# hiroharu-kato/neural_renderer

Measured on AMD Instinct MI355X. Metric: rasterize fwd+bwd Mpixels/sec @256x256 batch=64, higher is better.
Workload: dtype f32

## Files before the change

neural_renderer_amd/csrc/nr_forward.hip:

```cpp
#include "nr_device.h"

using namespace nr;

namespace {

constexpr size_t SMALL_LAUNCH_FACES = (size_t)16384 * 32;
constexpr int SMALL_AREA = 256;
constexpr int WAVE_AREA = 4096;
constexpr unsigned long long ZEMPTY = ~0ull;
constexpr int QSHARDS = 16;
constexpr int QSTRIDE = 32;

__device__ __forceinline__ unsigned depth_key(float zp)
{
    const unsigned u = __float_as_uint(zp + 0.0f);
    return (u & 0x80000000u) ? ~u : (u | 0x80000000u);
}

__device__ __forceinline__ unsigned long long zword(float zp, unsigned fn, int epoch)
{
    const unsigned long long k = depth_key(zp);
    return epoch < 0 ? (k << 32) | fn : ((unsigned long long)(unsigned)epoch << 56) | (k << 24) | fn;
}

// ... 350 lines not shown
            const int b = i / F;
            raster_candidates(
                g, (unsigned)(i - b * F), cd.n, (int)(threadIdx.x >> 6) * 64, 256,
                [&](int k, int &x, int &y) { return cand_pixel(cd, k, S, x, y); }, queue, S, near_d, far_d,
                zbuf + (size_t)b * S * S, epoch, touched, (size_t)b * S * S);
        }
    }
    wave_raster(faces, zbuf, wave_list, cnt, qcap, nshards, F, S, near_d, far_d, queue, epoch, touched);
}

enum ShadeMode { SHADE_CUBE = 0, SHADE_UV = 1, SHADE_CORNER = 2, SHADE_UV_SMOOTH = 3 };
__device__ __forceinline__ void load_background(const float *__restrict__ background, int bg_per_batch, int b, float (&bg)[3])
{
    const float *p = background + (bg_per_batch ? 3 * b : 0);
    bg[0] = p[0];
    bg[1] = p[1];
    bg[2] = p[2];
}

template <bool TS2>
struct CubeFace {
    float fz[3], lc[3];
    const float *texture;
    bool flip;
    float4 cube[TS2 ? 6 : 1];
};

template <bool TS2, bool SHARED = false>
__device__ __forceinline__ void load_cube_face(CubeFace<TS2> &c, int b, int fi, const float *__restrict__ faces,
                                               const float *__restrict__ zbase, const float *__restrict__ textures, int F,
                                               int ts, int fix_batch_z, const FaceLight &lit)
{
    const float *face = (fix_batch_z ? faces + (size_t)b * F * 9 : zbase) + (size_t)fi * 9;
    c.fz[0] = face[2]; c.fz[1] = face[5]; c.fz[2] = face[8];
    if constexpr (TS2) {
        c.flip = false;
        c.texture = textures + ((size_t)(SHARED ? 0 : b) * F + fi) * 24;
    } else {
        c.flip = lit.light && fi >= lit.tex_faces;
        c.texture = textures + ((size_t)(SHARED ? 0 : b) * (lit.light ? lit.tex_faces : F) + (c.flip ? fi - lit.tex_faces : fi)) * ts * ts * ts * 3;
        const float *lc = lit.light ? lit.light + ((size_t)b * F + fi) * 3 : face;
        c.lc[0] = lc[0]; c.lc[1] = lc[1]; c.lc[2] = lc[2];
    }
}

__device__ __forceinline__ void load_cube(CubeFace<true> &c)
{
#pragma unroll
    for (int k = 0; k < 6; k++) c.cube[k] = reinterpret_cast<const float4 *>(c.texture)[k];
}
__device__ __forceinline__ void load_cube(CubeFace<false> &) {}

__device__ __forceinline__ float quad_elem(const float4 &q, int k) { return k == 0 ? q.x : (k == 1 ? q.y : (k == 2 ? q.z : q.w)); }

__device__ __forceinline__ void store_taps(const Taps &t, int32_t *__restrict__ sampling_index_map,
                                           float *__restrict__ sampling_weight_map, size_t i)
{
    if (sampling_index_map) {
        int4 *p = reinterpret_cast<int4 *>(sampling_index_map + 8 * i);
        p[0] = make_int4(t.isc[0], t.isc[1], t.isc[2], t.isc[3]);
        p[1] = make_int4(t.isc[4], t.isc[5], t.isc[6], t.isc[7]);
    }
    if (sampling_weight_map) {
        float4 *p = reinterpret_cast<float4 *>(sampling_weight_map + 8 * i);
        p[0] = make_float4(t.w[0], t.w[1], t.w[2], t.w[3]);
        p[1] = make_float4(t.w[4], t.w[5], t.w[6], t.w[7]);
    }
}

template <bool TS2>
__device__ __forceinline__ void shade_cube(const CubeFace<TS2> &c, const float (&w)[3], float depth, int ts, double eps,
                                           bool lit, Taps &t, float (&rgb)[3], int32_t *__restrict__ sampling_index_map = nullptr,
                                           float *__restrict__ sampling_weight_map = nullptr, size_t i = 0)
{
    compute_taps(c.fz, w, depth, ts, eps, t, c.flip);
    store_taps(t, sampling_index_map, sampling_weight_map, i);
    if constexpr (TS2) {
        rgb[0] = rgb[1] = rgb[2] = 0.0f;
#pragma unroll
        for (int pn = 0; pn < 8; pn++) {
            const int b0 = pn & 1, b1 = (pn >> 1) & 1, b2 = pn >> 2;
            const int e = (b0 * 4 + b1 * 2 + b2) * 3;
#pragma unroll
            for (int k = 0; k < 3; k++) rgb[k] += t.w[pn] * quad_elem(c.cube[(e + k) >> 2], (e + k) & 3);
        }
    } else {
        sum_taps(c.texture, t, ts * ts * ts, rgb);
    }
    if (!TS2 && lit) {
        rgb[0] *= c.lc[0];
        rgb[1] *= c.lc[1];
        rgb[2] *= c.lc[2];
    }
}

template <int MODE>
__device__ __forceinline__ void shade_pixel(size_t i, int b, int fi, float w0, float w1, float w2, float depth,
                                            const float *__restrict__ faces, const float *__restrict__ zbase,
                                            const float *__restrict__ textures, float *__restrict__ rgb_map,
                                            int32_t *__restrict__ sampling_index_map,
                                            float *__restrict__ sampling_weight_map, const float (&bg)[3],
                                            float *__restrict__ alpha_map, int F, int ts, double eps, int fix_batch_z,
                                            const FaceLight &lit, const UVShade *uv = nullptr)
{
    if (alpha_map) alpha_map[i] = (fi >= 0) ? 1.0f : 0.0f;
    if (!rgb_map) return;
    float rgb[3];
    Taps t;
    constexpr bool UV = MODE == SHADE_UV || MODE == SHADE_UV_SMOOTH;
    if (MODE == SHADE_CORNER && fi >= 0) {
        const float *face = faces + ((size_t)b * F + fi) * 9;
        const float *cc = textures + ((size_t)b * F + fi) * 9;
        const float w[3] = {w0, w1, w2}, fz[3] = {face[2], face[5], face[8]};
        float d[3];
        corner_weights(fz, w, depth, d);
#pragma unroll
        for (int c = 0; c < 3; c++) {
            rgb[c] = (cc[c] * d[0] + cc[3 + c] * d[1]) + cc[6 + c] * d[2];
            rgb[c] = rgb[c] * 1.0f + 0.0f * bg[c];
        }
    } else if (UV && fi >= 0) {
        UVSample s;
        uv_locate(*uv, fi, lit.tex_faces, faces + ((size_t)b * F + fi) * 9, w0, w1, w2, depth, eps, s);
        uv_color(*uv, s, b, rgb);
        if (MODE == SHADE_UV_SMOOTH) {
            const float *face = faces + ((size_t)b * F + fi) * 9;
            const float w[3] = {w0, w1, w2}, fz[3] = {face[2], face[5], face[8]};
            float e[3];
            corner_weights(fz, w, depth, e);
            const float *lc = lit.light + ((size_t)b * F + fi) * 9;
#pragma unroll
            for (int c = 0; c < 3; c++) rgb[c] *= (lc[c] * e[0] + lc[3 + c] * e[1]) + lc[6 + c] * e[2];
        } else {
            const float *lc = lit.light + ((size_t)b * F + fi) * 3;
            rgb[0] *= lc[0];
            rgb[1] *= lc[1];
            rgb[2] *= lc[2];
        }
#pragma unroll
        for (int k = 0; k < 3; k++) rgb[k] = rgb[k] * 1.0f + 0.0f * bg[k];
    } else if (fi >= 0) {
        CubeFace<false> c;
        load_cube_face(c, b, fi, faces, zbase, textures, F, ts, fix_batch_z, lit);
        const float w[3] = {w0, w1, w2};
        shade_cube(c, w, depth, ts, eps, lit.light != nullptr, t, rgb, sampling_index_map, sampling_weight_map, i);
#pragma unroll
        for (int k = 0; k < 3; k++) rgb[k] = rgb[k] * 1.0f + 0.0f * bg[k];
    } else {
#pragma unroll
        for (int k = 0; k < 3; k++) rgb[k] = 0.0f * 0.0f + 1.0f * bg[k];
#pragma unroll
        for (int pn = 0; pn < 8; pn++) { t.isc[pn] = 0; t.w[pn] = 0.0f; }
    }
    float *o = rgb_map + 3 * i;
    o[0] = rgb[0];
    o[1] = rgb[1];
    o[2] = rgb[2];
    if (MODE == SHADE_CUBE && fi < 0) store_taps(t, sampling_index_map, sampling_weight_map, i);
}

__global__ __launch_bounds__(256) void k_shade(const float *__restrict__ faces, const float *__restrict__ zbase,
                                               const float *__restrict__ textures,
                                               const int32_t *__restrict__ face_index_map,
                                               const float *__restrict__ weight_map,
                                               const float *__restrict__ depth_map, float *__restrict__ rgb_map,
                                               int32_t *__restrict__ sampling_index_map,
                                               float *__restrict__ sampling_weight_map,
                                               const float *__restrict__ background, int bg_per_batch,
                                               float *__restrict__ alpha_map, int F, int S, int ts, double eps,
                                               int fix_batch_z, size_t n_pixels, FaceLight lit)
{
    const size_t i = (size_t)blockIdx.x * blockDim.x + threadIdx.x;
    if (i >= n_pixels) return;
    const int b = (int)(i / ((size_t)S * S));
    float bg[3] = {0.0f, 0.0f, 0.0f};
    if (rgb_map) load_background(background, bg_per_batch, b, bg);
    const int fi = face_index_map[i];
    float w0 = 0.0f, w1 = 0.0f, w2 = 0.0f, depth = 0.0f;
    if (rgb_map && fi >= 0) { w0 = weight_map[3 * i]; w1 = weight_map[3 * i + 1]; w2 = weight_map[3 * i + 2]; depth = depth_map[i]; }
    shade_pixel<SHADE_CUBE>(i, b, fi, w0, w1, w2, depth, faces, zbase, textures, rgb_map, sampling_index_map, sampling_weight_map,
                            bg, alpha_map, F, ts, eps, fix_batch_z, lit);
}

struct ResolveArgs {
    const float *faces;
    const unsigned long long *zbuf;
    int32_t *face_index_map;
    float *weight_map, *depth_map, *face_inv_map;
    unsigned char *visible_faces;
    int F, S;
    double near_d, far_d;
    size_t n_pixels;
    const float *zbase, *textures;
    float *rgb_map;
    const float *background;
    int bg_per_batch;
    float *alpha_map;
    int ts;
    double eps;
    int fix_batch_z, epoch;
    int *queue_counters;
    FaceLight lit;
    int sparse_weights;
    const unsigned char *touched;
};
struct ResolveArgsUV : ResolveArgs {
    UVShade uv;
};
template <int MODE> using ResolveArgsOf =
    typename std::conditional<MODE == SHADE_UV || MODE == SHADE_UV_SMOOTH, ResolveArgsUV, ResolveArgs>::type;

template <int MODE, bool TS2, bool SHARED = false>
__device__ __forceinline__ void resolve_pixel(const ResolveArgsOf<MODE> &a, size_t i, unsigned long long pk, const float (&bg)[3])
{
    constexpr bool CUBE = MODE == SHADE_CUBE;
    const float *__restrict__ faces = a.faces;
    const int S = a.S, F = a.F, epoch = a.epoch;
    int fn = -1;
    float zp = (float)a.far_d, w0 = 0.0f, w1 = 0.0f, w2 = 0.0f;
    int b = 0;
    float rgb[3];
    const bool hit = epoch < 0 ? pk != ZEMPTY : (int)(pk >> 56) == epoch;
    if (hit) {
        fn = epoch < 0 ? (int)(unsigned)(pk & 0xffffffffu) : (int)(unsigned)(pk & 0xffffffu);
        const size_t SS = (size_t)S * S;
        b = (int)(i / SS);
        const int pn = (int)(i - (size_t)b * SS);
        const int py = pn / S, px = pn - py * S;
        const float *f = faces + ((size_t)b * F + fn) * 9;
        const float fv[9] = {f[0], f[1], f[2], f[3], f[4], f[5], f[6], f[7], f[8]};
        CubeFace<TS2> c;
        if (CUBE && a.rgb_map) load_cube_face<TS2, SHARED>(c, b, fn, faces, a.zbase, a.textures, F, a.ts, a.fix_batch_z, a.lit);
        FaceGeo g;
        float inv[9];
        face_geo(fv, S, g, inv);
        if (CUBE && a.rgb_map) load_cube(c);
        eval_pixel(g, pixel_center_f(px, S), pixel_center_f(py, S), (float)px, (float)py, a.near_d, a.far_d, zp, w0, w1, w2);
        if (a.face_inv_map) {
            float *o = a.face_inv_map + 9 * i;
#pragma unroll
            for (int k = 0; k < 9; k++) o[k] = inv[k];
        }
        if (CUBE && a.rgb_map) {
            Taps t;
            const float w[3] = {w0, w1, w2};
            shade_cube(c, w, zp, a.ts, a.eps, a.lit.light != nullptr, t, rgb);
#pragma unroll
            for (int k = 0; k < 3; k++) rgb[k] = rgb[k] * 1.0f + 0.0f * bg[k];
        }
    } else {
#pragma unroll
        for (int k = 0; k < 3; k++) rgb[k] = 0.0f * 0.0f + 1.0f * bg[k];
    }
    a.face_index_map[i] = fn;
    if (a.depth_map) a.depth_map[i] = zp;
    if (a.weight_map && (hit || !a.sparse_weights)) {
        float *w = a.weight_map + 3 * i;
        w[0] = w0;
        w[1] = w1;
        w[2] = w2;
    }
    if (a.face_inv_map && !hit) {
        float *o = a.face_inv_map + 9 * i;
#pragma unroll
        for (int k = 0; k < 9; k++) o[k] = 0.0f;
    }
    if (hit && a.visible_faces) a.visible_faces[(size_t)b * F + fn] = 1;
    if constexpr (CUBE) {
        if (a.alpha_map) a.alpha_map[i] = hit ? 1.0f : 0.0f;
        if (a.rgb_map) {
            float *o = a.rgb_map + 3 * i;
            o[0] = rgb[0];
            o[1] = rgb[1];
            o[2] = rgb[2];
        }
    } else if (a.rgb_map || a.alpha_map) {
        const UVShade *uv = nullptr;
        if constexpr (MODE == SHADE_UV || MODE == SHADE_UV_SMOOTH) uv = &a.uv;
        shade_pixel<MODE>(i, b, fn, w0, w1, w2, zp, faces, a.zbase, a.textures, a.rgb_map, nullptr, nullptr, bg, a.alpha_map, F,
                          a.ts, a.eps, a.fix_batch_z, a.lit, uv);
    }
}

__device__ __forceinline__ void reset_queue_counters(const ResolveArgs &a)
{
    if (blockIdx.x == 0 && threadIdx.x < QSHARDS && a.epoch >= 0) {
        a.queue_counters[threadIdx.x * QSTRIDE] = -1;
        a.queue_counters[threadIdx.x * QSTRIDE + 1] = -1;
    }
}

template <int MODE, bool SHARED = false>
__global__ __launch_bounds__(256, 8) void k_resolve(ResolveArgsOf<MODE> a)
{
    const size_t i = (size_t)blockIdx.x * blockDim.x + threadIdx.x;
    reset_queue_counters(a);
    if (i >= a.n_pixels) return;
    float bg[3] = {0.0f, 0.0f, 0.0f};
    if (a.rgb_map) load_background(a.background, a.bg_per_batch, a.bg_per_batch ? (int)(i / ((size_t)a.S * a.S)) : 0, bg);
    const bool drawn = !a.touched || a.touched[i >> 6] == (unsigned char)a.epoch;
    resolve_pixel<MODE, false, SHARED>(a, i, drawn ? a.zbuf[i] : ZEMPTY, bg);
}

template <int MODE, bool TS2 = false, bool SHARED = false>
__global__ __launch_bounds__(256, 8) void k_resolve_quads(ResolveArgsOf<MODE> a)
{
    reset_queue_counters(a);
    const size_t i = (size_t)blockIdx.x * 256 + threadIdx.x, i0 = (size_t)blockIdx.x * 256 + 4 * threadIdx.x;
    const size_t last = a.n_pixels - 1;
    const unsigned char ep = (unsigned char)a.epoch;
    const bool filler = threadIdx.x < 64 && i0 < a.n_pixels;
    const unsigned char tq_read = a.touched[(filler ? i0 : min(i, last)) >> 6], ti_read = a.touched[min(i, last) >> 6];
    float bg[3] = {0.0f, 0.0f, 0.0f};
    if (a.rgb_map)
        load_background(a.background, a.bg_per_batch, a.bg_per_batch ? (int)(((size_t)blockIdx.x * 256) / ((size_t)a.S * a.S)) : 0, bg);
    const unsigned char tq = filler ? tq_read : ep, ti = i < a.n_pixels ? ti_read : (unsigned char)(ep + 1);
    unsigned long long pk = ZEMPTY;
    if (ti == ep) pk = a.zbuf[i];
    if (tq != ep) {
        reinterpret_cast<int4 *>(a.face_index_map)[i0 >> 2] = make_int4(-1, -1, -1, -1);
        const float zf = (float)a.far_d;
        if (a.depth_map) reinterpret_cast<float4 *>(a.depth_map)[i0 >> 2] = make_float4(zf, zf, zf, zf);
        const float4 zero = make_float4(0.0f, 0.0f, 0.0f, 0.0f);
        if (a.weight_map && !a.sparse_weights) {
            float4 *w = reinterpret_cast<float4 *>(a.weight_map + 3 * i0);
            w[0] = zero; w[1] = zero; w[2] = zero;
        }
        if (a.face_inv_map) {
            float4 *o = reinterpret_cast<float4 *>(a.face_inv_map + 9 * i0);
#pragma unroll
            for (int k = 0; k < 9; k++) o[k] = zero;
        }
        if (a.alpha_map) reinterpret_cast<float4 *>(a.alpha_map)[i0 >> 2] = zero;
        if (a.rgb_map) {
            float c[3];
#pragma unroll
            for (int k = 0; k < 3; k++) c[k] = 0.0f * 0.0f + 1.0f * bg[k];
            float4 *o = reinterpret_cast<float4 *>(a.rgb_map + 3 * i0);
            o[0] = make_float4(c[0], c[1], c[2], c[0]);
            o[1] = make_float4(c[1], c[2], c[0], c[1]);
            o[2] = make_float4(c[2], c[0], c[1], c[2]);
        }
    }
    if (ti == ep) resolve_pixel<MODE, TS2, SHARED>(a, i, pk, bg);
}

}

NR_API int nr_version(void) { return NR_VERSION; }

NR_API const char *nr_error_string(int code)
{
    switch (code) {
        case 0: return "success";
        case NR_E_NULL: return "nr: a required pointer is NULL";
        case NR_E_SIZE: return "nr: size out of range";
        case NR_E_WORKSPACE: return "nr: workspace missing or too small";
        case NR_E_MODE: return "nr: nothing to do / inconsistent optional arguments";
        case NR_E_INDEX: return "nr: a vertex index lies outside [0, num_vertices)";
        default: return code > 0 ? hipGetErrorString((hipError_t)code) : "nr: unknown error";
    }
}

namespace {
struct FwdLayout {
    size_t zbuf_off, list_off, count_off, touch_off, total;
};
size_t queue_shard_capacity(size_t n_faces, int faces_per_wave, int nshards)
{
    const size_t per_wg = (size_t)4 * faces_per_wave, n_wg = (n_faces + per_wg - 1) / per_wg;
    return (n_wg + nshards - 1) / nshards * per_wg;
}

FwdLayout fwd_layout(int B, int F, int S)
{
    FwdLayout L;
    const size_t n = (size_t)B * F, P = (size_t)B * S * S;
    L.zbuf_off = 0;
    L.count_off = L.zbuf_off + P * sizeof(unsigned long long);
    L.list_off = align_up(L.count_off + (size_t)QSHARDS * QSTRIDE * sizeof(int), 256);
    L.touch_off = align_up(L.list_off + 2 * (n + (size_t)QSHARDS * 256) * sizeof(int), 256);
    L.total = L.touch_off + (P + 63) / 64;
    return L;
}
}

NR_API size_t nr_forward_workspace_bytes(int32_t B, int32_t F, int32_t S)
{
    if (check_sizes(B, F, S)) return 0;
    return fwd_layout(B, F, S).total;
}

namespace {
int run_forward(const float *faces, int32_t *face_index_map, float *weight_map, float *depth_map, float *face_inv_map,
                unsigned char *visible_faces, int B, int F, int S, double near, double far, void *workspace,
                size_t workspace_bytes, hipStream_t st, const float *faces_z_ref, const float *textures, float *rgb_map,
                const float *background, int bg_per_batch, float *alpha_map, int ts, double eps, int fix_batch_z,
                int flags = 0, const FaceLight &lit = FaceLight(), const UVShade *uv = nullptr, bool corner = false,
                bool corner_light = false, bool shared_cubes = false)
{
    if (!faces || !face_index_map) return NR_E_NULL;
    if (int e = check_sizes(B, F, S)) return e;
    const FwdLayout L = fwd_layout(B, F, S);
    if (!workspace || workspace_bytes < L.total) return NR_E_WORKSPACE;
    const size_t n = (size_t)B * F, P = (size_t)B * S * S;
    unsigned char *ws = (unsigned char *)workspace;
    unsigned long long *zbuf = (unsigned long long *)(ws + L.zbuf_off);
    int *n_large = (int *)(ws + L.count_off);
    int *large_list = (int *)(ws + L.list_off);

    int epoch = -1;
    if ((flags & NR_FLAG_ZBUF_EPOCH) && F < (1 << 24)) {
        epoch = (flags >> 8) & 0xff;
        if (epoch > 254) return NR_E_MODE;
    } else {
        if (int he = fill_bytes(zbuf, 0xff, P * sizeof(unsigned long long) + (size_t)QSHARDS * QSTRIDE * sizeof(int), st)) return he;
    }
    const bool small_launch = n < SMALL_LAUNCH_FACES;
    const int nshards = small_launch ? 1 : QSHARDS;
    const int qcap = (int)queue_shard_capacity(n, small_launch ? 16 : 64, nshards);
    int *wave_list = large_list + (size_t)nshards * qcap;
    unsigned char *touched = epoch >= 0 ? ws + L.touch_off : nullptr;
    {
        const bool pow2 = (S & (S - 1)) == 0, small = small_launch;
#define NR_FACE_RASTER(P, FC, G)                                                                                           \
    hipLaunchKernelGGL((k_face_raster<P, FC, G>), dim3((unsigned)((n + 4 * FC - 1) / (4 * FC))), dim3(256), 0, st, faces, zbuf, \
                       large_list, wave_list, n_large, qcap, nshards, visible_faces, (int)n, F, S, near, far, epoch, touched)
        if (small) { if (pow2) NR_FACE_RASTER(true, 16, 4); else NR_FACE_RASTER(false, 16, 4); }
        else { if (pow2) NR_FACE_RASTER(true, 64, 16); else NR_FACE_RASTER(false, 64, 16); }
#undef NR_FACE_RASTER
    }
    const unsigned queue_wgs = (unsigned)(n / 256 < 256 ? 256 : (n / 256 > 2048 ? 2048 : n / 256));
    hipLaunchKernelGGL(k_large_raster, dim3(queue_wgs), dim3(256), 0, st, faces, zbuf, large_list, wave_list, n_large, qcap, nshards,
                       F, S, near, far, epoch, touched);
    ResolveArgs ra;
    ra.faces = faces; ra.zbuf = zbuf; ra.face_index_map = face_index_map; ra.weight_map = weight_map; ra.depth_map = depth_map;
    ra.face_inv_map = face_inv_map; ra.visible_faces = visible_faces; ra.F = F; ra.S = S; ra.near_d = near; ra.far_d = far;
    ra.n_pixels = P; ra.zbase = faces_z_ref ? faces_z_ref : faces; ra.textures = textures; ra.rgb_map = rgb_map;
    ra.background = background; ra.bg_per_batch = bg_per_batch; ra.alpha_map = alpha_map; ra.ts = ts; ra.eps = eps;
    ra.fix_batch_z = fix_batch_z; ra.epoch = epoch; ra.queue_counters = n_large; ra.lit = lit;
    ra.sparse_weights = (flags & NR_FLAG_SPARSE_WEIGHT_MAP) ? 1 : 0; ra.touched = touched;
    const uintptr_t align = (uintptr_t)face_index_map | (uintptr_t)weight_map | (uintptr_t)depth_map | (uintptr_t)face_inv_map |
                            (uintptr_t)rgb_map | (uintptr_t)alpha_map;
    const bool quads = touched && S % 2 == 0 && (align & 15) == 0 && (!(rgb_map && bg_per_batch) || ((size_t)S * S) % 256 == 0);
    const dim3 grid((unsigned)((P + 255) / 256));
    if (uv) {
        ResolveArgsUV rau;
        static_cast<ResolveArgs &>(rau) = ra;
        rau.uv = *uv;
        if (corner_light) {
            if (quads) hipLaunchKernelGGL(k_resolve_quads<SHADE_UV_SMOOTH>, grid, dim3(256), 0, st, rau);
            else hipLaunchKernelGGL(k_resolve<SHADE_UV_SMOOTH>, grid, dim3(256), 0, st, rau);
        } else if (quads) {
            hipLaunchKernelGGL(k_resolve_quads<SHADE_UV>, grid, dim3(256), 0, st, rau);
        } else {
            hipLaunchKernelGGL(k_resolve<SHADE_UV>, grid, dim3(256), 0, st, rau);
        }
    } else if (corner) {
        if (quads) hipLaunchKernelGGL(k_resolve_quads<SHADE_CORNER>, grid, dim3(256), 0, st, ra);
        else hipLaunchKernelGGL(k_resolve<SHADE_CORNER>, grid, dim3(256), 0, st, ra);
    } else if (shared_cubes) {
        if (quads && rgb_map && !lit.light && ts == 2 && (float)(1.0 - eps) < 1.0f && ((uintptr_t)textures & 15) == 0)
            hipLaunchKernelGGL((k_resolve_quads<SHADE_CUBE, true, true>), grid, dim3(256), 0, st, ra);
        else if (quads) hipLaunchKernelGGL((k_resolve_quads<SHADE_CUBE, false, true>), grid, dim3(256), 0, st, ra);
        else hipLaunchKernelGGL((k_resolve<SHADE_CUBE, true>), grid, dim3(256), 0, st, ra);
    } else if (quads && rgb_map && !lit.light && ts == 2 && (float)(1.0 - eps) < 1.0f && ((uintptr_t)textures & 15) == 0) {
        hipLaunchKernelGGL((k_resolve_quads<SHADE_CUBE, true>), grid, dim3(256), 0, st, ra);
    } else if (quads) {
        hipLaunchKernelGGL(k_resolve_quads<SHADE_CUBE>, grid, dim3(256), 0, st, ra);
    } else {
        hipLaunchKernelGGL(k_resolve<SHADE_CUBE>, grid, dim3(256), 0, st, ra);
    }
    return launch_status();
}
}

NR_API int nr_forward_face_index_map(const float *faces, int32_t *face_index_map, float *weight_map, float *depth_map,
                                     float *face_inv_map, uint8_t *visible_faces, int32_t B, int32_t F, int32_t S,
                                     double near, double far, void *workspace, size_t workspace_bytes, void *stream)
{
    return run_forward(faces, face_index_map, weight_map, depth_map, face_inv_map, visible_faces, B, F, S, near, far,
                       workspace, workspace_bytes, (hipStream_t)stream, nullptr, nullptr, nullptr, nullptr, 0, nullptr, 0,
                       0.0, 0);
}

NR_API int nr_forward_rasterize(const float *faces, const float *faces_z_ref, const float *textures,
                                int32_t *face_index_map, float *weight_map, float *depth_map, float *rgb_map,
                                float *alpha_map, uint8_t *visible_faces, const float *background, int32_t bg_per_batch,
                                int32_t B, int32_t F, int32_t S, int32_t ts, double near, double far, double eps,
                                int32_t flags, void *workspace, size_t workspace_bytes, void *stream)
{
    return nr_forward_rasterize_lit(nullptr, faces, faces_z_ref, textures, face_index_map, weight_map, depth_map, rgb_map,
                                    alpha_map, visible_faces, background, bg_per_batch, B, F, S, ts, near, far, eps, flags,
                                    workspace, workspace_bytes, stream);
}

int nr::face_light_args(const nr_face_light *lit, int F, bool backward, FaceLight &out)
{
    out = FaceLight();
    if (!lit) return 0;
    if (!lit->light) return NR_E_NULL;
    if (lit->texture_faces < 1 || (lit->texture_faces != F && 2 * (int64_t)lit->texture_faces != F)) return NR_E_SIZE;
    out.light = lit->light;
    out.tex_faces = lit->texture_faces;
    if (backward) {
        out.textures = lit->textures;
        out.grad_light = lit->grad_light;
        if (out.grad_light && !out.textures) return NR_E_NULL;
    }
    return 0;
}

NR_API int nr_forward_rasterize_lit(const nr_face_light *lit, const float *faces, const float *faces_z_ref,
                                    const float *textures, int32_t *face_index_map, float *weight_map, float *depth_map,
                                    float *rgb_map, float *alpha_map, uint8_t *visible_faces, const float *background,
                                    int32_t bg_per_batch, int32_t B, int32_t F, int32_t S, int32_t ts, double near,
                                    double far, double eps, int32_t flags, void *workspace, size_t workspace_bytes,
                                    void *stream)
{
    if (rgb_map) {
        if (!textures || !background) return NR_E_NULL;
        if (ts < 2 || ts > 1024) return NR_E_SIZE;
    }
    FaceLight fl;
    if (int e = face_light_args(rgb_map ? lit : nullptr, F, false, fl)) return e;
    return run_forward(faces, face_index_map, weight_map, depth_map, nullptr, visible_faces, B, F, S, near, far,
                       workspace, workspace_bytes, (hipStream_t)stream, faces_z_ref, textures, rgb_map, background,
                       bg_per_batch, alpha_map, ts, eps, (flags & NR_FLAG_FIX_TEXTURE_BATCH_Z) ? 1 : 0, flags, fl, nullptr, false,
                       false, rgb_map && (flags & NR_FLAG_SHARED_TEXTURES));
}

int nr::uv_images_args(const nr_face_light *lit, const nr_uv_images *uv, int B, int F, FaceLight &fl, UVShade &out)
{
    out = UVShade();
    if (!lit || !uv) return NR_E_NULL;
    if (int e = face_light_args(lit, F, false, fl)) return e;
    fl.grad_light = lit->grad_light;
    if (!uv->images || !uv->image_table || !uv->faces_uv || !uv->face_image || !uv->base) return NR_E_NULL;
    if (uv->texture_size < 2 || uv->texture_size > 1024 || uv->num_images < 1 || uv->num_pixels < 1 ||
        uv->num_pixels > 0x7ffffffe)
        return NR_E_SIZE;
    if (uv->image_batch != 1 && uv->image_batch != B) return NR_E_SIZE;
    out.images = uv->images;
    out.table = uv->image_table;
    out.faces_uv = uv->faces_uv;
    out.face_image = uv->face_image;
    out.base = uv->base;
    out.ts = uv->texture_size;
    out.M = uv->num_images;
    out.P = uv->num_pixels;
    out.shared = uv->image_batch == 1 ? 1 : 0;
    return 0;
}

NR_API int nr_forward_rasterize_uv(const nr_face_light *lit, const nr_uv_images *uv, const float *faces,
                                   int32_t *face_index_map, float *weight_map, float *depth_map, float *rgb_map,
                                   float *alpha_map, uint8_t *visible_faces, const float *background, int32_t bg_per_batch,
                                   int32_t B, int32_t F, int32_t S, double near, double far, double eps, int32_t flags,
                                   void *workspace, size_t workspace_bytes, void *stream)
{
    if (!rgb_map || !background) return NR_E_NULL;
    FaceLight fl;
    UVShade us;
    if (int e = uv_images_args(lit, uv, B, F, fl, us)) return e;
    return run_forward(faces, face_index_map, weight_map, depth_map, nullptr, visible_faces, B, F, S, near, far,
                       workspace, workspace_bytes, (hipStream_t)stream, nullptr, nullptr, rgb_map, background,
                       bg_per_batch, alpha_map, us.ts, eps, 1, flags, fl, &us);
}

int nr::uv_smooth_args(const nr_corner_light *lit, const nr_uv_images *uv, int B, int F, FaceLight &fl, UVShade &out)
{
    if (!lit) return NR_E_NULL;
    const nr_face_light as_face = {lit->light, lit->texture_faces, nullptr, lit->grad_light};
    return uv_images_args(&as_face, uv, B, F, fl, out);
}

NR_API int nr_forward_rasterize_uv_smooth(const nr_corner_light *lit, const nr_uv_images *uv, const float *faces,
                                          int32_t *face_index_map, float *weight_map, float *depth_map, float *rgb_map,
                                          float *alpha_map, uint8_t *visible_faces, const float *background,
                                          int32_t bg_per_batch, int32_t B, int32_t F, int32_t S, double near, double far,
                                          double eps, int32_t flags, void *workspace, size_t workspace_bytes, void *stream)
{
    if (!rgb_map || !background) return NR_E_NULL;
    FaceLight fl;
    UVShade us;
    if (int e = uv_smooth_args(lit, uv, B, F, fl, us)) return e;
    return run_forward(faces, face_index_map, weight_map, depth_map, nullptr, visible_faces, B, F, S, near, far,
                       workspace, workspace_bytes, (hipStream_t)stream, nullptr, nullptr, rgb_map, background,
                       bg_per_batch, alpha_map, us.ts, eps, 1, flags, fl, &us, false, true);
}

NR_API int nr_forward_rasterize_corner(const float *corner_colors, const float *faces, int32_t *face_index_map,
                                       float *weight_map, float *depth_map, float *rgb_map, float *alpha_map,
                                       uint8_t *visible_faces, const float *background, int32_t bg_per_batch, int32_t B,
                                       int32_t F, int32_t S, double near, double far, int32_t flags, void *workspace,
                                       size_t workspace_bytes, void *stream)
{
    if (!corner_colors || !rgb_map || !background) return NR_E_NULL;
    return run_forward(faces, face_index_map, weight_map, depth_map, nullptr, visible_faces, B, F, S, near, far,
                       workspace, workspace_bytes, (hipStream_t)stream, nullptr, corner_colors, rgb_map, background,
                       bg_per_batch, alpha_map, 2, 0.0, 1, flags, FaceLight(), nullptr, true);
}

NR_API int nr_forward_texture_sampling(const float *faces, const float *faces_z_ref, const float *textures,
                                       const int32_t *face_index_map, const float *weight_map, const float *depth_map,
                                       float *rgb_map, int32_t *sampling_index_map, float *sampling_weight_map,
                                       const float *background, int32_t bg_per_batch, float *alpha_map, int32_t B,
                                       int32_t F, int32_t S, int32_t ts, double eps, int32_t flags, void *stream)
{
    if (!face_index_map) return NR_E_NULL;
    if (!rgb_map && !alpha_map) return NR_E_MODE;
    if (flags & NR_FLAG_SHARED_TEXTURES) return NR_E_MODE;
    if (int e = check_sizes(B, F, S)) return e;
    if (rgb_map) {
        if (!faces || !textures || !weight_map || !depth_map || !background) return NR_E_NULL;
        if (ts < 2 || ts > 1024) return NR_E_SIZE;
        if ((sampling_index_map == nullptr) != (sampling_weight_map == nullptr)) return NR_E_MODE;
    }
    const size_t n = (size_t)B * S * S;
    hipLaunchKernelGGL(k_shade, dim3((unsigned)((n + 255) / 256)), dim3(256), 0, (hipStream_t)stream, faces,
                       faces_z_ref ? faces_z_ref : faces, textures, face_index_map, weight_map, depth_map, rgb_map,
                       sampling_index_map, sampling_weight_map, background, bg_per_batch, alpha_map, F, S, ts, eps,
                       (flags & NR_FLAG_FIX_TEXTURE_BATCH_Z) ? 1 : 0, n, FaceLight());
    return launch_status();
}
```

neural_renderer_amd/csrc/nr_k6_lists.h:

```cpp

__global__ __launch_bounds__(256) void k_mark_visible(const int32_t *__restrict__ fi_map,
                                                      unsigned char *__restrict__ flags, int F, int SS, size_t P)
{
    const size_t i = (size_t)blockIdx.x * blockDim.x + threadIdx.x;
    if (i >= P) return;
    const int fi = fi_map[i];
    if (fi >= 0) flags[(i / SS) * F + fi] = 1;
}

__device__ __forceinline__ void emit_visible(int b, int fn, int pos, int F, int S, const float *__restrict__ faces,
                                             int *__restrict__ vis_list, unsigned *__restrict__ rng,
                                             double *__restrict__ scratch, int *band_count, int n_bands, int W,
                                             int *line_diff = nullptr)
{
    vis_list[(size_t)b * F + pos] = fn;
    const float *f = faces + ((size_t)b * F + fn) * 9;
    const float fs = (float)S;
    float px[3], py[3];
#pragma unroll
    for (int k = 0; k < 3; k++) { px[k] = to_pixel(f[3 * k], fs); py[k] = to_pixel(f[3 * k + 1], fs); }
    unsigned *r0 = rng + (((size_t)b * 2 + 0) * F + pos) * 3, *r1 = rng + (((size_t)b * 2 + 1) * F + pos) * 3;
#pragma unroll
    for (int e = 0; e < 3; e++) {
        const unsigned ra = edge_range(px[e], px[(e + 1) % 3], S), rb = edge_range(py[e], py[(e + 1) % 3], S);
        r0[e] = ra;
        r1[e] = rb;
#pragma unroll
        for (int axis = 0; axis < 2; axis++) {
            const unsigned r = axis ? rb : ra;
            const int lo = (int)(r & 0xffffu), hi = (int)(r >> 16);
            if (line_diff) {
                if (lo <= hi) {
                    atomicAdd(line_diff + axis * (S + 1) + lo, 1);
                    atomicAdd(line_diff + axis * (S + 1) + hi + 1, -1);
                }
                continue;
            }
            for (int band = lo / W; band * W <= hi; ++band)
                atomicAdd(band_count + axis * n_bands + band, min(hi, band * W + W - 1) - max(lo, band * W) + 1);
        }
    }
    double2 *z = reinterpret_cast<double2 *>(scratch + ((size_t)b * F + pos) * 6);
    z[0] = z[1] = z[2] = make_double2(0.0, 0.0);
}

__device__ __forceinline__ void zero_face(float *__restrict__ o)
{
#pragma unroll
    for (int k = 0; k < 9; k++) o[k] = 0.0f;
}

constexpr int VIS_CHUNK = 1024;
constexpr int SMALL_CHUNKS = 16;

__device__ __forceinline__ int chunk_flags_before(const unsigned char *flags, int b, int F, int chunk)
{
    int part = 0;
    for (int c = 0, tid = threadIdx.x; c < chunk; ++c) part += __popcll(__ballot(flags[(size_t)b * F + c * VIS_CHUNK + tid] != 0));
    return part;
}
__device__ __forceinline__ unsigned long long chunk_rank(bool v, int part, int *s_part, int *s_wcnt, int &off, int &own)
{
    const int tid = threadIdx.x, lane = tid & 63, wave = tid >> 6;
    const unsigned long long m = __ballot(v);
    if (lane == 0) { s_part[wave] = part; s_wcnt[wave] = __popcll(m); }
    __syncthreads();
    off = own = 0;
    for (int w = 0; w < VIS_CHUNK / 64; ++w) {
        off += s_part[w];
        if (w < wave) off += s_wcnt[w];
        own += s_wcnt[w];
    }
    return m;
}
__device__ __forceinline__ int chunk_rank_total(int own, const int *s_part)
{
    int base = 0;
    for (int w = 0; w < VIS_CHUNK / 64; ++w) base += s_part[w];
    return base + own;
}

__global__ __launch_bounds__(VIS_CHUNK) void k_compact_par(const unsigned char *__restrict__ flags,
                                                           int *__restrict__ vis_list, int *__restrict__ vis_count,
                                                           int *__restrict__ slot_of, int F, int n_chunks,
                                                           const float *__restrict__ faces, unsigned *__restrict__ rng,
                                                           double *__restrict__ scratch, int S,
                                                           int *__restrict__ chunk_band, int n_bands, int W,
                                                           int *__restrict__ band_cursor, float *__restrict__ zero_faces,
                                                           int zero_listed, int use_diff, int *__restrict__ ticket)
{
    extern __shared__ int s_band[];
    __shared__ int s_wcnt[VIS_CHUNK / 64];
    __shared__ int s_part[VIS_CHUNK / 64];
    const int b = blockIdx.y, chunk = blockIdx.x, tid = threadIdx.x, lane = tid & 63, wave = tid >> 6;
    for (int i = tid; i < 2 * n_bands; i += VIS_CHUNK) s_band[i] = 0;
    int *s_diff = use_diff ? s_band + 2 * n_bands : nullptr;
    if (use_diff)
        for (int i = tid; i < 2 * (S + 1); i += VIS_CHUNK) s_diff[i] = 0;
    const int part = chunk_flags_before(flags, b, F, chunk), fn = chunk * VIS_CHUNK + tid;
    const bool v = fn < F && flags[(size_t)b * F + fn] != 0;
    int off, own;
    const unsigned long long m = chunk_rank(v, part, s_part, s_wcnt, off, own);
    if (fn < F) {
        const int before = off + __popcll(m & ((1ull << lane) - 1ull));
        slot_of[(size_t)b * F + fn] = v ? before : -1;
        if (v) emit_visible(b, fn, before, F, S, faces, vis_list, rng, scratch, s_band, n_bands, W, s_diff);
        if (zero_faces && (!v || zero_listed)) zero_face(zero_faces + ((size_t)b * F + fn) * 9);
    }
    __syncthreads();
    if (use_diff) {
        const int n2 = 2 * (S + 1), per = (n2 + VIS_CHUNK - 1) / VIS_CHUNK, i0 = tid * per, i1 = min(n2, i0 + per);
        int local = 0;
        for (int i = i0; i < i1; ++i) local += s_diff[i];
        const int inc = wave_incl_scan(local, lane);
        __syncthreads();
        if (lane == 63) s_wcnt[wave] = inc;
        __syncthreads();
        int run = inc - local;
        for (int w = 0; w < wave; ++w) run += s_wcnt[w];
        for (int i = i0; i < i1; ++i) {
            run += s_diff[i];
            s_diff[i] = run;
        }
        __syncthreads();
        for (int i = tid; i < 2 * n_bands; i += VIS_CHUNK) {
            const int axis = i >= n_bands, band = i - axis * n_bands;
            int c = 0;
            for (int l = band * W; l < min(S, band * W + W); ++l) c += s_diff[axis * (S + 1) + l];
            s_band[i] = c;
        }
        __syncthreads();
    }
    int *row = chunk_band + ((size_t)b * n_chunks + chunk) * 2 * n_bands;
    for (int i = tid; i < 2 * n_bands; i += VIS_CHUNK) row[i] = s_band[i];
    if (chunk == 0)
        for (int i = tid; i < 2 * n_bands; i += VIS_CHUNK) band_cursor[(size_t)b * 2 * n_bands + i] = 0;
    if (chunk == n_chunks - 1 && tid == 0) vis_count[b] = chunk_rank_total(own, s_part);
    if (chunk == 0 && b == 0 && tid == 0) *ticket = 0;
}

__global__ __launch_bounds__(VIS_CHUNK) void k_list_visible(const unsigned char *__restrict__ flags,
                                                            int *__restrict__ vis_list, int *__restrict__ vis_count, int F,
                                                            int n_chunks)
{
    __shared__ int s_wcnt[VIS_CHUNK / 64];
    __shared__ int s_part[VIS_CHUNK / 64];
    const int b = blockIdx.y, chunk = blockIdx.x, tid = threadIdx.x, lane = tid & 63;
    const int part = chunk_flags_before(flags, b, F, chunk), fn = chunk * VIS_CHUNK + tid;
    const bool v = fn < F && flags[(size_t)b * F + fn] != 0;
    int off, own;
    const unsigned long long m = chunk_rank(v, part, s_part, s_wcnt, off, own);
    if (v) vis_list[(size_t)b * F + off + __popcll(m & ((1ull << lane) - 1ull))] = fn;
    if (chunk == n_chunks - 1 && tid == 0) vis_count[b] = chunk_rank_total(own, s_part);
}

__global__ __launch_bounds__(VIS_CHUNK) void k_count_visible(const unsigned char *__restrict__ flags,
                                                             int *__restrict__ chunk_count, int F, int n_chunks,
                                                             int *__restrict__ band_lines, int n_bands)
{
    __shared__ int s_wcnt[VIS_CHUNK / 64];
    const int b = blockIdx.y, chunk = blockIdx.x, tid = threadIdx.x, lane = tid & 63, wave = tid >> 6;
    for (int i = chunk * VIS_CHUNK + tid; i < 2 * n_bands; i += n_chunks * VIS_CHUNK) band_lines[(size_t)b * 2 * n_bands + i] = 0;
    const int fn = chunk * VIS_CHUNK + tid;
    const bool v = fn < F && flags[(size_t)b * F + fn] != 0;
    const unsigned long long m = __ballot(v);
    if (lane == 0) s_wcnt[wave] = __popcll(m);
    __syncthreads();
    if (tid == 0) {
        int tot = 0;
        for (int w = 0; w < VIS_CHUNK / 64; ++w) tot += s_wcnt[w];
        chunk_count[(size_t)b * n_chunks + chunk] = tot;
    }
}

__global__ __launch_bounds__(VIS_CHUNK) void k_compact_visible(const unsigned char *__restrict__ flags,
                                                               const int *__restrict__ chunk_count,
                                                               int *__restrict__ vis_list, int *__restrict__ vis_count,
                                                               int *__restrict__ slot_of, int F, int n_chunks,
                                                               const float *__restrict__ faces,
                                                               unsigned *__restrict__ rng, double *__restrict__ scratch,
                                                               int S, int *__restrict__ band_lines, int n_bands, int W,
                                                               int lds_counters, float *__restrict__ zero_faces,
                                                               int zero_listed)
{
    extern __shared__ int s_band[];
    __shared__ int s_wcnt[VIS_CHUNK / 64];
    __shared__ int s_part[VIS_CHUNK / 64];
    const int b = blockIdx.y, chunk = blockIdx.x, tid = threadIdx.x;
    if (lds_counters)
        for (int i = tid; i < 2 * n_bands; i += VIS_CHUNK) s_band[i] = 0;
    int part = 0;
    for (int c = tid; c < chunk; c += VIS_CHUNK) part += chunk_count[(size_t)b * n_chunks + c];
#pragma unroll
    for (int o = 32; o > 0; o >>= 1) part += __shfl_xor(part, o, WAVE);
    const int fn = chunk * VIS_CHUNK + tid;
    const bool v = fn < F && flags[(size_t)b * F + fn] != 0;
    int off, own;
    const unsigned long long m = chunk_rank(v, part, s_part, s_wcnt, off, own);
    if (fn < F) {
        const int before = off + __popcll(m & ((1ull << (tid & 63)) - 1ull));
        slot_of[(size_t)b * F + fn] = v ? before : -1;
        if (zero_faces && (!v || zero_listed)) zero_face(zero_faces + ((size_t)b * F + fn) * 9);
        if (v)
            emit_visible(b, fn, before, F, S, faces, vis_list, rng, scratch,
                         lds_counters ? s_band : band_lines + (size_t)b * 2 * n_bands, n_bands, W);
    }
    if (lds_counters) {
        __syncthreads();
        for (int i = tid; i < 2 * n_bands; i += VIS_CHUNK) {
            const int c = s_band[i];
            if (c) atomicAdd(band_lines + (size_t)b * 2 * n_bands + i, c);
        }
    }
    if (chunk == n_chunks - 1 && tid == 0) vis_count[b] = chunk_rank_total(own, s_part);
}

template <int NT>
__device__ __forceinline__ int block_excl_scan(int v, int *s_tmp, int *total)
{
    const int tid = threadIdx.x, lane = tid & 63, wave = tid >> 6;
    const int inc = wave_incl_scan(v, lane);
    if (lane == 63) s_tmp[wave] = inc;
    __syncthreads();
    int woff = 0, tot = 0;
    for (int w = 0; w < NT / 64; ++w) {
        const int c = s_tmp[w];
        if (w < wave) woff += c;
        tot += c;
    }
    __syncthreads();
    *total = tot;
    return woff + inc - v;
}

__device__ __forceinline__ double signed_eps(float dist, unsigned eps_hi, unsigned eps_lo)
{
    return __hiloint2double((int)((0.0f < dist) ? eps_hi : (eps_hi ^ 0x80000000u)), (int)eps_lo);
}

__global__ __launch_bounds__(256, 8) void k_line_setup(LineSetupArgs a)
{
    const SlotImage w = image_fastest(blockIdx.x, a.grid_y);
    line_setup_body(a, w.bx, w.by);
}

__device__ __forceinline__ void band_prefix(const int *cnt, int n2, int *__restrict__ start_out, int *__restrict__ cursor_out,
                                            int *__restrict__ ok_out, size_t cap)
{
    if (threadIdx.x >= 64) return;
    const int lane = threadIdx.x, per = (n2 + 63) / 64;
    int local = 0;
    for (int i = lane * per; i < min(n2, (lane + 1) * per); ++i) local += cnt[i];
    const int inc = wave_incl_scan(local, lane);
    int run = inc - local;
    for (int i = lane * per; i < min(n2, (lane + 1) * per); ++i) {
        start_out[i] = run;
        cursor_out[i] = 0;
        run += cnt[i];
    }
    const int total = __shfl(inc, 63, WAVE);
    if (lane == 0) *ok_out = ((size_t)total <= cap) ? 1 : 0;
}

__global__ __launch_bounds__(256) void k_band_scan(const int *__restrict__ band_lines, int *__restrict__ band_start,
                                                   int *__restrict__ band_cursor, int *__restrict__ lines_ok, int n_bands,
                                                   size_t cap, int force_scan, int *__restrict__ ticket)
{
    if (blockIdx.x == 0 && threadIdx.x == 0) *ticket = 0;
    const size_t o = (size_t)blockIdx.x * 2 * n_bands;
    band_prefix(band_lines + o, 2 * n_bands, band_start + o, band_cursor + o, lines_ok + blockIdx.x, force_scan ? 0 : cap);
}

__global__ __launch_bounds__(256) void k_band_total(const int *__restrict__ chunk_band, int n_sum, int *__restrict__ band_lines,
                                                    int *__restrict__ band_start, int *__restrict__ lines_ok, int n_bands)
{
    const int b = blockIdx.x, n2 = 2 * n_bands;
    const int *rows = chunk_band + (size_t)b * n_sum * n2;
    for (int i = threadIdx.x; i < n2; i += blockDim.x) {
        int t = 0;
        for (int c = 0; c < n_sum; ++c) t += rows[(size_t)c * n2 + i];
        band_lines[(size_t)b * n2 + i] = t;
        band_start[(size_t)b * n2 + i] = 0;
    }
    if (threadIdx.x == 0) lines_ok[b] = 0;
}
```

Baseline: 16510.

## Coalesce background fills and per-chunk zeroing of face and scratch buffers

```diff
diff --git a/neural_renderer_amd/csrc/nr_forward.hip b/neural_renderer_amd/csrc/nr_forward.hip
--- a/neural_renderer_amd/csrc/nr_forward.hip
+++ b/neural_renderer_amd/csrc/nr_forward.hip
@@ -676,44 +676,61 @@
     resolve_pixel<MODE, false, SHARED>(a, i, drawn ? a.zbuf[i] : ZEMPTY, bg);
 }
 
+template <int WPQ>
+__device__ __forceinline__ void fill_block(float *map, unsigned tw, unsigned ep, size_t n_pixels, float4 r0, float4 r1, float4 r2)
+{
+    float4 *o = reinterpret_cast<float4 *>(map) + (size_t)blockIdx.x * (64 * WPQ);
+    const size_t left = (n_pixels >> 2) * WPQ - (size_t)blockIdx.x * (64 * WPQ);
+    const int l = threadIdx.x, l3 = l % 3;
+#pragma unroll
+    for (int k = 0; k < WPQ; k++) {
+        const int w = 64 * k + l, r = l3 + k % 3;
+        const bool p0 = r == 0 || r == 3, p1 = r == 1 || r == 4;
+        if ((size_t)w < left && ((tw >> (8 * (w / (16 * WPQ)))) & 0xffu) != ep)
+            o[w] = make_float4(p0 ? r0.x : (p1 ? r1.x : r2.x), p0 ? r0.y : (p1 ? r1.y : r2.y), p0 ? r0.z : (p1 ? r1.z : r2.z),
+                               p0 ? r0.w : (p1 ? r1.w : r2.w));
+    }
+}
+
 template <int MODE, bool TS2 = false, bool SHARED = false>
 __global__ __launch_bounds__(256, 8) void k_resolve_quads(ResolveArgsOf<MODE> a)
 {
     reset_queue_counters(a);
     const size_t i = (size_t)blockIdx.x * 256 + threadIdx.x, i0 = (size_t)blockIdx.x * 256 + 4 * threadIdx.x;
-    const size_t last = a.n_pixels - 1;
-    const unsigned char ep = (unsigned char)a.epoch;
-    const bool filler = threadIdx.x < 64 && i0 < a.n_pixels;
-    const unsigned char tq_read = a.touched[(filler ? i0 : min(i, last)) >> 6], ti_read = a.touched[min(i, last) >> 6];
+    const unsigned ep = (unsigned char)a.epoch;
+    const size_t seg0 = (size_t)blockIdx.x * 4, n_seg = (a.n_pixels + 63) >> 6;
+    unsigned tw;
+    if (seg0 + 4 <= n_seg) {
+        tw = *reinterpret_cast<const unsigned *>(a.touched + seg0);
+    } else {
+        tw = 0;
+#pragma unroll
+        for (int s = 0; s < 4; s++) tw |= (seg0 + s < n_seg ? (unsigned)a.touched[min(seg0 + s, n_seg - 1)] : ep) << (8 * s);
+    }
     float bg[3] = {0.0f, 0.0f, 0.0f};
     if (a.rgb_map)
         load_background(a.background, a.bg_per_batch, a.bg_per_batch ? (int)(((size_t)blockIdx.x * 256) / ((size_t)a.S * a.S)) : 0, bg);
-    const unsigned char tq = filler ? tq_read : ep, ti = i < a.n_pixels ? ti_read : (unsigned char)(ep + 1);
+    const bool wave0 = threadIdx.x < 64, filler = wave0 && i0 < a.n_pixels;
+    const unsigned tq = filler ? (tw >> (8 * (threadIdx.x >> 4))) & 0xffu : ep;
+    const unsigned ti = i < a.n_pixels ? (tw >> (8 * (threadIdx.x >> 6))) & 0xffu : ep + 1;
     unsigned long long pk = ZEMPTY;
     if (ti == ep) pk = a.zbuf[i];
-    if (tq != ep) {
-        reinterpret_cast<int4 *>(a.face_index_map)[i0 >> 2] = make_int4(-1, -1, -1, -1);
-        const float zf = (float)a.far_d;
-        if (a.depth_map) reinterpret_cast<float4 *>(a.depth_map)[i0 >> 2] = make_float4(zf, zf, zf, zf);
+    if (wave0 && tw != ep * 0x01010101u) {
         const float4 zero = make_float4(0.0f, 0.0f, 0.0f, 0.0f);
-        if (a.weight_map && !a.sparse_weights) {
-            float4 *w = reinterpret_cast<float4 *>(a.weight_map + 3 * i0);
-            w[0] = zero; w[1] = zero; w[2] = zero;
-        }
-        if (a.face_inv_map) {
-            float4 *o = reinterpret_cast<float4 *>(a.face_inv_map + 9 * i0);
-#pragma unroll
-            for (int k = 0; k < 9; k++) o[k] = zero;
-        }
-        if (a.alpha_map) reinterpret_cast<float4 *>(a.alpha_map)[i0 >> 2] = zero;
+        if (tq != ep) {
+            reinterpret_cast<int4 *>(a.face_index_map)[i0 >> 2] = make_int4(-1, -1, -1, -1);
+            const float zf = (float)a.far_d;
+            if (a.depth_map) reinterpret_cast<float4 *>(a.depth_map)[i0 >> 2] = make_float4(zf, zf, zf, zf);
+        }
+        if (a.weight_map && !a.sparse_weights) fill_block<3>(a.weight_map, tw, ep, a.n_pixels, zero, zero, zero);
+        if (a.face_inv_map) fill_block<9>(a.face_inv_map, tw, ep, a.n_pixels, zero, zero, zero);
+        if (tq != ep && a.alpha_map) reinterpret_cast<float4 *>(a.alpha_map)[i0 >> 2] = zero;
         if (a.rgb_map) {
             float c[3];
 #pragma unroll
             for (int k = 0; k < 3; k++) c[k] = 0.0f * 0.0f + 1.0f * bg[k];
-            float4 *o = reinterpret_cast<float4 *>(a.rgb_map + 3 * i0);
-            o[0] = make_float4(c[0], c[1], c[2], c[0]);
-            o[1] = make_float4(c[1], c[2], c[0], c[1]);
-            o[2] = make_float4(c[2], c[0], c[1], c[2]);
+            fill_block<3>(a.rgb_map, tw, ep, a.n_pixels, make_float4(c[0], c[1], c[2], c[0]), make_float4(c[1], c[2], c[0], c[1]),
+                          make_float4(c[2], c[0], c[1], c[2]));
         }
     }
     if (ti == ep) resolve_pixel<MODE, TS2, SHARED>(a, i, pk, bg);
diff --git a/neural_renderer_amd/csrc/nr_k6_lists.h b/neural_renderer_amd/csrc/nr_k6_lists.h
--- a/neural_renderer_amd/csrc/nr_k6_lists.h
+++ b/neural_renderer_amd/csrc/nr_k6_lists.h
@@ -10,8 +10,7 @@
 
 __device__ __forceinline__ void emit_visible(int b, int fn, int pos, int F, int S, const float *__restrict__ faces,
                                              int *__restrict__ vis_list, unsigned *__restrict__ rng,
-                                             double *__restrict__ scratch, int *band_count, int n_bands, int W,
-                                             int *line_diff = nullptr)
+                                             int *band_count, int n_bands, int W, int *line_diff = nullptr)
 {
     vis_list[(size_t)b * F + pos] = fn;
     const float *f = faces + ((size_t)b * F + fn) * 9;
@@ -40,18 +39,33 @@
                 atomicAdd(band_count + axis * n_bands + band, min(hi, band * W + W - 1) - max(lo, band * W) + 1);
         }
     }
-    double2 *z = reinterpret_cast<double2 *>(scratch + ((size_t)b * F + pos) * 6);
-    z[0] = z[1] = z[2] = make_double2(0.0, 0.0);
-}
-
-__device__ __forceinline__ void zero_face(float *__restrict__ o)
-{
-#pragma unroll
-    for (int k = 0; k < 9; k++) o[k] = 0.0f;
 }
 
 constexpr int VIS_CHUNK = 1024;
 constexpr int SMALL_CHUNKS = 16;
+
+__device__ __forceinline__ void zero_chunk_faces(float *__restrict__ zero_faces, int b, int F, int chunk, int zero_listed,
+                                                 const unsigned char *s_vis)
+{
+    const int f0 = chunk * VIS_CHUNK, n = 9 * min(VIS_CHUNK, F - f0), tid = threadIdx.x;
+    float *o = zero_faces + ((size_t)b * F + f0) * 9;
+    if (zero_listed) {
+        const int head = min(n, (int)((4 - (((uintptr_t)o >> 2) & 3)) & 3)), nw = (n - head) >> 2, tail = n - head - 4 * nw;
+        float4 *o4 = reinterpret_cast<float4 *>(o + head);
+        for (int w = tid; w < nw; w += VIS_CHUNK) o4[w] = make_float4(0.0f, 0.0f, 0.0f, 0.0f);
+        if (tid < head) o[tid] = 0.0f;
+        if (tid < tail) o[head + 4 * nw + tid] = 0.0f;
+    } else {
+        for (int d = tid; d < n; d += VIS_CHUNK)
+            if (!s_vis[d / 9]) o[d] = 0.0f;
+    }
+}
+
+__device__ __forceinline__ void zero_chunk_sums(double *__restrict__ scratch, int b, int F, int base, int own)
+{
+    double2 *z = reinterpret_cast<double2 *>(scratch + ((size_t)b * F + base) * 6);
+    for (int w = threadIdx.x; w < 3 * own; w += VIS_CHUNK) z[w] = make_double2(0.0, 0.0);
+}
 
 __device__ __forceinline__ int chunk_flags_before(const unsigned char *flags, int b, int F, int chunk)
 {
@@ -92,6 +106,7 @@
     extern __shared__ int s_band[];
     __shared__ int s_wcnt[VIS_CHUNK / 64];
     __shared__ int s_part[VIS_CHUNK / 64];
+    __shared__ unsigned char s_vis[VIS_CHUNK];
     const int b = blockIdx.y, chunk = blockIdx.x, tid = threadIdx.x, lane = tid & 63, wave = tid >> 6;
     for (int i = tid; i < 2 * n_bands; i += VIS_CHUNK) s_band[i] = 0;
     int *s_diff = use_diff ? s_band + 2 * n_bands : nullptr;
@@ -99,14 +114,16 @@
         for (int i = tid; i < 2 * (S + 1); i += VIS_CHUNK) s_diff[i] = 0;
     const int part = chunk_flags_before(flags, b, F, chunk), fn = chunk * VIS_CHUNK + tid;
     const bool v = fn < F && flags[(size_t)b * F + fn] != 0;
+    s_vis[tid] = v;
     int off, own;
     const unsigned long long m = chunk_rank(v, part, s_part, s_wcnt, off, own);
     if (fn < F) {
         const int before = off + __popcll(m & ((1ull << lane) - 1ull));
         slot_of[(size_t)b * F + fn] = v ? before : -1;
-        if (v) emit_visible(b, fn, before, F, S, faces, vis_list, rng, scratch, s_band, n_bands, W, s_diff);
-        if (zero_faces && (!v || zero_listed)) zero_face(zero_faces + ((size_t)b * F + fn) * 9);
-    }
+        if (v) emit_visible(b, fn, before, F, S, faces, vis_list, rng, s_band, n_bands, W, s_diff);
+    }
+    if (zero_faces) zero_chunk_faces(zero_faces, b, F, chunk, zero_listed, s_vis);
+    zero_chunk_sums(scratch, b, F, chunk_rank_total(0, s_part), own);
     __syncthreads();
     if (use_diff) {
         const int n2 = 2 * (S + 1), per = (n2 + VIS_CHUNK - 1) / VIS_CHUNK, i0 = tid * per, i1 = min(n2, i0 + per);
@@ -186,6 +203,7 @@
     extern __shared__ int s_band[];
     __shared__ int s_wcnt[VIS_CHUNK / 64];
     __shared__ int s_part[VIS_CHUNK / 64];
+    __shared__ unsigned char s_vis[VIS_CHUNK];
     const int b = blockIdx.y, chunk = blockIdx.x, tid = threadIdx.x;
     if (lds_counters)
         for (int i = tid; i < 2 * n_bands; i += VIS_CHUNK) s_band[i] = 0;
@@ -195,16 +213,18 @@
     for (int o = 32; o > 0; o >>= 1) part += __shfl_xor(part, o, WAVE);
     const int fn = chunk * VIS_CHUNK + tid;
     const bool v = fn < F && flags[(size_t)b * F + fn] != 0;
+    s_vis[tid] = v;
     int off, own;
     const unsigned long long m = chunk_rank(v, part, s_part, s_wcnt, off, own);
     if (fn < F) {
         const int before = off + __popcll(m & ((1ull << (tid & 63)) - 1ull));
         slot_of[(size_t)b * F + fn] = v ? before : -1;
-        if (zero_faces && (!v || zero_listed)) zero_face(zero_faces + ((size_t)b * F + fn) * 9);
         if (v)
-            emit_visible(b, fn, before, F, S, faces, vis_list, rng, scratch,
-                         lds_counters ? s_band : band_lines + (size_t)b * 2 * n_bands, n_bands, W);
-    }
+            emit_visible(b, fn, before, F, S, faces, vis_list, rng, lds_counters ? s_band : band_lines + (size_t)b * 2 * n_bands,
+                         n_bands, W);
+    }
+    if (zero_faces) zero_chunk_faces(zero_faces, b, F, chunk, zero_listed, s_vis);
+    zero_chunk_sums(scratch, b, F, chunk_rank_total(0, s_part), own);
     if (lds_counters) {
         __syncthreads();
         for (int i = tid; i < 2 * n_bands; i += VIS_CHUNK) {
```

Result: faster. 16730 (median of 5 runs) (+1.4%).
